# zyang1580/PDA

Hardware: AMD Instinct MI355X
Metric: users/sec full-catalogue top-K@50 (eval) (higher is better)
Workload: dtype f32; 1 GPU; C3: synthetic 1000000 users x 200000 items, d=128, PDA condition ((elu+1)*pop^0.22) head, masked top-K@50; ranks_seen=1

## Files before the change

include/pda_hip_experimental.h:

```cpp
#ifndef PDA_HIP_EXPERIMENTAL_H
#define PDA_HIP_EXPERIMENTAL_H

#include "pda_hip.h"

#ifdef __cplusplus
extern "C" {
#endif

int pda_score_topk_huge_splits(int n_users_blk, int n_items_local, int d);

int pda_topk_kth_value(const uint64_t* keys, int n_splits, int n_users_blk, int K, int pos, float* out, void* stream);
int pda_topk_remap_items(uint64_t* keys, size_t n_keys, const int32_t* gid, int n_gid, void* stream);
int pda_topk_seed_bounds(const uint64_t* keys, int n_splits, int n_users_blk, int K, int m, float* bounds, void* stream);
int pda_topk_seed_counts(const uint64_t* keys, int n_splits, int n_users_blk, int K, const float* bounds, int n_thr, int32_t* counts,
                         void* stream);
int pda_topk_seed_pick(const float* bounds, const int32_t* counts, int n_thr, int n_users_blk, int K, float* seed, void* stream);
int pda_topk_seed_refine(const uint64_t* keys, int n_splits, int n_users_blk, int K, float* lo, float* hi, float* mid, int32_t* counts,
                         int mode, void* stream);
int pda_score_topk4_phase_f32(const float* U, const float* I_shard, const void* prep, const float* pop_shard, const int32_t* users,
                              int n_users_blk, int item_offset, int n_items_local, int d, const int64_t* hist_indptr,
                              const int32_t* hist_indices, int hist_row_mode, int K, int head, int early_stop, int n_splits,
                              int phase, int warm_tiles, const float* seed, uint64_t* out_keys, void* workspace, void* stream);
int pda_score_topk4_phase_bf16(const uint16_t* U, const uint16_t* I_shard, const void* prep, const float* pop_shard,
                               const int32_t* users, int n_users_blk, int item_offset, int n_items_local, int d,
                               const int64_t* hist_indptr, const int32_t* hist_indices, int hist_row_mode, int K, int head,
                               int early_stop, int n_splits, int phase, int warm_tiles, const float* seed, uint64_t* out_keys,
                               void* workspace, void* stream);
int pda_score_topk4_phase_image_offsets(int n_users_blk, int n_items_local, int d, int n_splits, size_t* offs);
int pda_score_topk4_phase_user_image(const void* U, int bf16, const int32_t* users, int n_users_blk, int d, void* ufrag, float* unorm,
                                     void* stream);
int pda_score_topk4_phase_mask_table(const void* prep, int n_items_local, int d, int item_offset, const int64_t* hist_indptr,
                                     const int32_t* hist_indices, int n_rows, uint32_t* table, void* stream);
int pda_score_topk4_phase_masked_f32(const float* U, const float* I_shard, const void* prep, const float* pop_shard, const int32_t* users,
                                     int n_users_blk, int item_offset, int n_items_local, int d, const int64_t* hist_indptr,
                                     const int32_t* hist_indices, int hist_row_mode, int K, int head, int early_stop, int n_splits,
                                     const uint32_t* mask_table, int mask_table_rows, uint64_t* out_keys, void* workspace, void* stream);
int pda_score_topk4_phase_masked_bf16(const uint16_t* U, const uint16_t* I_shard, const void* prep, const float* pop_shard, const int32_t* users,
                                      int n_users_blk, int item_offset, int n_items_local, int d, const int64_t* hist_indptr,
                                      const int32_t* hist_indices, int hist_row_mode, int K, int head, int early_stop, int n_splits,
                                      const uint32_t* mask_table, int mask_table_rows, uint64_t* out_keys, void* workspace, void* stream);
int pda_score_topk4_phase_mask_rows(const void* prep, const int32_t* users, int n_users_blk, int item_offset, int n_items_local, int d,
                                    const int64_t* hist_indptr, const int32_t* hist_indices, int hist_row_mode, int warm_tiles, uint32_t* out,
                                    void* stream);
int pda_score_topk4_phase_mask_offsets(int n_users_blk, int n_items_local, int d, int n_splits, size_t* offs);
#define PDA_SWEEP_WARM_ONE_KERNEL 2048

size_t pda_triplet_plan_bytes(int B);
size_t pda_triplet_plan_large_workspace_bytes(int B);
int pda_triplet_plan_large(const int32_t* users, const int32_t* pos, const int32_t* neg, int B, void* plan, void* workspace, void* stream);
size_t pda_bpr_step_plan_scratch_bytes(int B, int d);
int pda_triplet_plan(const int32_t* users, const int32_t* pos, const int32_t* neg, int B, int n_batches, void* plans, void* stream);
int pda_bpr_step_plan_f32(float* U, float* I, const int32_t* users, const int32_t* pos, const int32_t* neg, const float* pos_pop,
                          const float* neg_pop, int B, int d, float regs, float reg_div, float lr, const void* plan, float* scratch,
                          int exact, float* loss_acc, void* stream);
int pda_bpr_step_plan_bf16(uint16_t* U_bf16, uint16_t* I_bf16, float* U_master, float* I_master, const int32_t* users,
                           const int32_t* pos, const int32_t* neg, const float* pos_pop, const float* neg_pop, int B, int d,
                           float regs, float reg_div, float lr, const void* plan, float* scratch, float* loss_acc, void* stream);

int pda_sort_triplets_by_pos(int32_t* users, int32_t* pos, int32_t* neg, float* pos_pop, float* neg_pop, int B,
                             void* stream);

int pda_group_triplets_by_pos(int32_t* users, int32_t* pos, int32_t* neg, float* pos_pop, float* neg_pop, int B,
                              void* stream);

int pda_adam_mark_rows(const int32_t* users, const int32_t* pos, const int32_t* neg, int B, uint32_t* touched_u, uint32_t* touched_i, void* stream);
int pda_adam_dense_sweep3_f32(float* var_a, float* m_a, float* v_a, float* g_a, size_t rows_a, uint32_t* touched_a, float* var_b, float* m_b, float* v_b,
                              float* g_b, size_t rows_b, uint32_t* touched_b, int d, float lr_t, float beta1, float beta2, float eps, void* stream);

int pda_adam_rows_f32(float* var, float* m, float* v, float* g, const int32_t* rows, int n_rows, int d, float lr_t,
                      float beta1, float beta2, float eps, void* stream);

int pda_adam_lazy_f32(int phase, float* U, float* mU, float* vU, float* gU, int32_t* lastU, float* I, float* mI, float* vI,
                      float* gI, int32_t* lastI, const int32_t* users, const int32_t* pos, const int32_t* neg, int B, int d, int t,
                      const float* lr_tab, float beta1, float beta2, float eps, void* stream);
int pda_adam_lazy_sync_f32(float* var, float* m, float* v, int32_t* last, size_t n_rows, int d, int t, const float* lr_tab,
                           float beta1, float beta2, float eps, void* stream);
int pda_adam_lazy_dev_f32(int phase, float* U, float* mU, float* vU, float* gU, int32_t* lastU, float* I, float* mI, float* vI,
// ... 42 lines not shown
```

pda_amd/_lib.py:

```python
from __future__ import annotations

import ctypes as C
import os

_HERE = os.path.dirname(os.path.abspath(__file__))
LIB_PATH = os.environ.get("PDA_HIP_LIB") or os.path.join(_HERE, "csrc", "libpda_hip.so")

ABI_VERSION = 2
HEAD_RAW, HEAD_POP = 0, 1
HIST_BY_BLOCK_ROW, HIST_BY_USER_ID = 0, 1
UPD_NONE, UPD_SGD_FUSED, UPD_DENSE_GRAD = 0, 1, 2
UPD_ANY_ORDER = 0x100
UPD_USERS_DISTINCT = 0x200
ADAM_REPLAY_FAST = 0x10
MAX_K = 64
TOPK_CAP = 60

_vp, _i, _f, _u64, _sz = C.c_void_p, C.c_int, C.c_float, C.c_uint64, C.c_size_t

class ScorePlan(C.Structure):
    _fields_ = [("path", _i), ("sweep_mode", _i), ("n_splits", _i), ("early_stop", _i), ("order", _i), ("prep_with_pop", _i),
                ("workspace_bytes", _sz), ("keys_rows", _sz)]


# ... 24 lines not shown
    "pda_item_prep_bf16": (_i, [_vp, _i, _i, _vp, _vp]),
    "pda_score_topk_bf16": (_i, [_vp, _vp, _vp, _vp, _vp, _i, _i, _i, _i, _vp, _vp, _i, _i, _i, _i, _vp, _vp, _vp]),
    "pda_item_prep_ordered_bf16_bytes": (_sz, [_i, _i]),
    "pda_item_prep_ordered_bf16": (_i, [_vp, _vp, _vp, _i, _i, _vp, _vp]),
    "pda_score_topk_ordered_bf16": (_i, [_vp, _vp, _vp, _vp, _vp, _i, _i, _i, _i, _vp, _vp, _vp, _i, _i, _i, _i, _i, _vp, _vp, _vp]),
    "pda_item_prep4_bytes": (_sz, [_i, _i]),
    "pda_item_prep4_f32": (_i, [_vp, _vp, _vp, _i, _i, _vp, _vp]),
    "pda_item_prep4_bf16": (_i, [_vp, _vp, _vp, _i, _i, _vp, _vp]),
    "pda_item_prep7_f32": (_i, [_vp, _vp, _i, _i, _vp, _vp]),
    "pda_item_prep7_bf16": (_i, [_vp, _vp, _i, _i, _vp, _vp]),
    "pda_item_prep4_check": (_i, [_vp, _i, _i, _vp]),
    "pda_score_topk4_auto_splits": (_i, [_i, _i, _i]),
    "pda_score_topk4_f32": (_i, [_vp, _vp, _vp, _vp, _vp, _i, _i, _i, _i, _vp, _vp, _i, _i, _i, _i, _i, _vp, _vp, _vp]),
    "pda_score_topk4_bf16": (_i, [_vp, _vp, _vp, _vp, _vp, _i, _i, _i, _i, _vp, _vp, _i, _i, _i, _i, _i, _vp, _vp, _vp]),
    "pda_peak_mfma_flops_per_launch": (C.c_double, [_i]),
    "pda_peak_mfma_bf16": (_i, [_vp, _i, _vp]),
    "pda_peak_mfma_bf16_const": (_i, [_vp, _i, _vp]),
    "pda_peak_mfma_lds_flops_per_launch": (C.c_double, [_i]),
    "pda_peak_mfma_lds_bf16": (_i, [_vp, _sz, _vp, _i, _vp]),
    "pda_peak_copy": (_i, [_vp, _vp, _sz, _vp]),
    "pda_topk_kth_value": (_i, [_vp, _i, _i, _i, _i, _vp, _vp]),
    "pda_topk_remap_items": (_i, [_vp, _sz, _vp, _i, _vp]),
    "pda_topk_seed_refine": (_i, [_vp, _i, _i, _i, _vp, _vp, _vp, _vp, _i, _vp]),
    "pda_topk_seed_bounds": (_i, [_vp, _i, _i, _i, _i, _vp, _vp]),
    "pda_topk_seed_counts": (_i, [_vp, _i, _i, _i, _vp, _i, _vp, _vp]),
    "pda_topk_seed_pick": (_i, [_vp, _vp, _i, _i, _i, _vp, _vp]),
    "pda_score_topk4_phase_f32": (_i, [_vp, _vp, _vp, _vp, _vp, _i, _i, _i, _i, _vp, _vp, _i, _i, _i, _i, _i, _i, _i, _vp, _vp, _vp, _vp]),
    "pda_score_topk4_phase_bf16": (_i, [_vp, _vp, _vp, _vp, _vp, _i, _i, _i, _i, _vp, _vp, _i, _i, _i, _i, _i, _i, _i, _vp, _vp, _vp, _vp]),
    "pda_score_topk4_phase_image_offsets": (_i, [_i, _i, _i, _i, _vp]),
    "pda_score_topk4_phase_user_image": (_i, [_vp, _i, _vp, _i, _i, _vp, _vp, _vp]),
    "pda_score_topk4_phase_mask_table": (_i, [_vp, _i, _i, _i, _vp, _vp, _i, _vp, _vp]),
    "pda_score_topk4_phase_mask_rows": (_i, [_vp, _vp, _i, _i, _i, _i, _vp, _vp, _i, _i, _vp, _vp]),
    "pda_score_topk4_phase_mask_offsets": (_i, [_i, _i, _i, _i, _vp]),
    "pda_score_topk4_phase_masked_f32": (_i, [_vp, _vp, _vp, _vp, _vp, _i, _i, _i, _i, _vp, _vp, _i, _i, _i, _i, _i, _vp, _i, _vp, _vp, _vp]),
    "pda_score_topk4_phase_masked_bf16": (_i, [_vp, _vp, _vp, _vp, _vp, _i, _i, _i, _i, _vp, _vp, _i, _i, _i, _i, _i, _vp, _i, _vp, _vp, _vp]),
    "pda_score_topk_plan": (_i, [_i, _i, _i, _i, _i, _i, _i, _i, _vp]),
    "pda_score_topk_huge_splits": (_i, [_i, _i, _i]),
    "pda_score_topk7_workspace_bytes": (_sz, [_i, _i, _i]),
    "pda_score_topk7_f32": (_i, [_vp, _vp, _vp, _vp, _i, _i, _i, _i, _vp, _vp, _i, _i, _i, _vp, _vp, _vp]),
    "pda_score_topk7_bf16": (_i, [_vp, _vp, _vp, _vp, _i, _i, _i, _i, _vp, _vp, _i, _i, _i, _vp, _vp, _vp]),
    "pda_topk_merge": (_i, [_vp, _i, _i, _i, _vp, _vp, _vp, _vp, _vp, _vp, _i, _vp]),
    "pda_bpr_step_f32": (_i, [_vp, _vp, _vp, _vp, _vp, _vp, _vp, _i, _i, _f, _f, _f, _i, _vp, _vp, _vp, _vp, _vp, _vp, _vp]),
    "pda_triplet_plan_bytes": (_sz, [_i]),
    "pda_bpr_step_plan_scratch_bytes": (_sz, [_i, _i]),
    "pda_triplet_plan": (_i, [_vp, _vp, _vp, _i, _i, _vp, _vp]),
    "pda_triplet_plan_large_workspace_bytes": (_sz, [_i]),
    "pda_triplet_plan_large": (_i, [_vp, _vp, _vp, _i, _vp, _vp, _vp]),
    "pda_bpr_step_plan_f32": (_i, [_vp, _vp, _vp, _vp, _vp, _vp, _vp, _i, _i, _f, _f, _f, _vp, _vp, _i, _vp, _vp]),
    "pda_bpr_step_plan_bf16": (_i, [_vp, _vp, _vp, _vp, _vp, _vp, _vp, _vp, _vp, _i, _i, _f, _f, _f, _vp, _vp, _vp, _vp]),
    "pda_sgd_apply_f32": (_i, [_vp, _vp, _vp, _vp, _vp, _vp, _vp, _vp, _i, _i, _f, _vp]),
    "pda_bpr_step_shard_f32": (_i, [_vp, _vp, _i, _vp, _vp, _vp, _vp, _vp, _i, _i, _f, _f, _f, _f, _vp, _i, _vp, _vp, _vp]),
    "pda_apply_user_grads_f32": (_i, [_vp, _vp, _vp, _i, _i, _i, _f, _vp]),
    "pda_bpr_step_bf16": (_i, [_vp, _vp, _vp, _vp, _vp, _vp, _vp, _vp, _vp, _i, _i, _f, _f, _f, _i, _vp, _vp, _vp, _vp, _vp, _vp, _vp]),
    "pda_refresh_rows_bf16": (_i, [_vp, _vp, _vp, _i, _i, _vp]),
    "pda_group_triplets_by_pos": (_i, [_vp, _vp, _vp, _vp, _vp, _i, _vp]),
    "pda_sort_triplets_by_pos": (_i, [_vp, _vp, _vp, _vp, _vp, _i, _vp]),
    "pda_adam_dense_sweep_f32": (_i, [_vp, _vp, _vp, _vp, _sz, _f, _f, _f, _f, _vp]),
    "pda_adam_dense_sweep2_f32": (_i, [_vp, _vp, _vp, _vp, _sz, _vp, _vp, _vp, _vp, _sz, _f, _f, _f, _f, _vp]),
    "pda_adam_mark_rows": (_i, [_vp, _vp, _vp, _i, _vp, _vp, _vp]),
    "pda_adam_dense_sweep3_f32": (_i, [_vp, _vp, _vp, _vp, _sz, _vp, _vp, _vp, _vp, _vp, _sz, _vp, _i, _f, _f, _f, _f, _vp]),
    "pda_score_dense_f32": (_i, [_vp, _vp, _vp, _vp, _i, _vp, _i, _i, _i, _vp, _vp]),
    "pda_adam_dense_sweep4_f32": (_i, [_vp, _vp, _vp, _vp, _sz, _vp, _vp, _vp, _vp, _vp, _sz, _vp, _i, _i, _f, _f, _f, _f, _i, _vp]),
    "pda_adam_step_f32": (_i, [_vp, _vp, _vp, _vp, _vp, _sz, _vp, _vp, _vp, _vp, _vp, _sz, _vp, _vp, _vp, _vp, _vp, _i, _i, _f, _f, _i, _f, _f, _f, _f,
                               _i, _i, _vp, _vp]),
    "pda_adam_rows_f32": (_i, [_vp, _vp, _vp, _vp, _vp, _i, _i, _f, _f, _f, _f, _vp]),
    "pda_adam_lazy_f32": (_i, [_i] + [_vp] * 13 + [_i, _i, _i, _vp, _f, _f, _f, _vp]),
# ... 121 lines not shown
```

pda_amd/csrc/pda_score_topk_v4.hip:

```cpp
#include "pda_v4_shared.h"
#include <cstdlib>
#include <type_traits>

using namespace pda_topk;

namespace {

constexpr int kCap4 = 57;
constexpr int kRing4 = 128;
constexpr int kWarmTiles = 4;
constexpr int kMainWaves = 8;
#ifndef PDA_W4_ABL
#define PDA_W4_ABL 0
#endif
#ifdef PDA_V4_PROF
__device__ unsigned long long pda_prof4[24];
#define PROF_T0(v) const long long v = __builtin_readcyclecounter()
#define PROF_T1(v, slot) prof[slot] += (unsigned long long)(__builtin_readcyclecounter() - v)
#define PROF_INC(slot, x) prof[slot] += (unsigned long long)(x)
#define PROF_FLUSH(first, last) do { if (lane == 0) for (int pq = (first); pq <= (last); ++pq) atomicAdd(&pda_prof4[pq], prof[pq]); } while (0)
#else
#define PROF_T0(v) do {} while (0)
#define PROF_T1(v, slot) do {} while (0)
#define PROF_INC(slot, x) do {} while (0)
// ... 680 lines not shown
        } else if (rb < g.n_users_blk && lane < K) {
            const uint64_t k = lane < c ? buf[lane] : 0ull;
            g.out_keys[((size_t)split * g.n_users_blk + rb) * K + lane] = k;
        }
    }
    if (g.kth_ws != nullptr) {
        pda_wave_sync();
        const int rb0 = utile * kUserTile + wave * 32, nv = max(0, min(32, g.n_users_blk - rb0));
        if (lane < nv) {
            const uint64_t kl = my_lists[(size_t)lane * CAP + (K - 1)];
            g.kth_ws[(size_t)split * g.n_users_blk + rb0 + lane] = cntl[wave * 32 + lane] >= K ? pda_unordf((uint32_t)(kl >> 32)) : -INFINITY;
        }
        uint64_t* ob = g.out_keys + ((size_t)split * g.n_users_blk + rb0) * K;
        const int q64 = 64 / K, r64 = 64 % K;
        int rr = lane / K, p = lane % K;
        for (int i = lane; i < nv * K; i += 64) {
            ob[i] = p < cntl[wave * 32 + rr] ? my_lists[(size_t)rr * CAP + p] : 0ull;
            rr += q64;
            p += r64;
            if (p >= K) { p -= K; ++rr; }
        }
    }
    if (g.pred_ws != nullptr && lane < 32) {
        const int rb = utile * kUserTile + wave * 32 + lane;
        if (rb < g.n_users_blk) {
            g.pred_ws[2 * (size_t)rb] = predt[wave * 32 + lane];
            g.pred_ws[2 * (size_t)rb + 1] = nul[wave * 32 + lane];
        }
    }
}

constexpr int kWS5Waves = 8, kWS5Threads = 64 * kWS5Waves;
constexpr int kWarmPos = 64 * kWarmTiles;
constexpr size_t warm_score5_lds(int d) { return (size_t)kWarmPos * d * 4 + kWarmPos * 8 + (size_t)kWS5Waves * 32 * 2 * kWarmTiles * 4; }

template <int D, bool BF>
__global__ void __launch_bounds__(kWS5Threads) warm_score5_kernel(Args4 g) {
    extern __shared__ __attribute__((aligned(16))) unsigned char smem[];
    constexpr int RB = row_bytes(D);
    constexpr int NC = D / 8;
    constexpr int CPR4 = D / 4;
    float* Bt = reinterpret_cast<float*>(smem);
    float* popw = Bt + kWarmPos * D;
    int* idw = reinterpret_cast<int*>(popw + kWarmPos);
    unsigned* hmask = reinterpret_cast<unsigned*>(idw + kWarmPos);

    const int tid = threadIdx.x, lane = tid & 63, wave = tid >> 6;
    const int j = lane & 31, h = lane >> 5;
    const int nwarm = g.warm_tiles;
    const int npos = 64 * nwarm;
    for (int p = tid; p < npos; p += kWS5Threads) {
        const float* tl = reinterpret_cast<const float*>(g.rows + (size_t)p * RB + 2 * D + 32);
        popw[p] = tl[0];
        idw[p] = reinterpret_cast<const int*>(tl)[1];
    }
    __syncthreads();
    for (int id = tid; id < npos * CPR4; id += kWS5Threads) {
        const int jj = id / CPR4, ch = id % CPR4;
        *reinterpret_cast<f32x4*>(Bt + jj * D + 4 * (ch ^ swz<D>(jj & 31))) = pda_load4<BF>(g.I, (size_t)idw[jj] * D + 4 * ch);
    }
    if (blockIdx.x == 0) {
        for (int p = tid; p < kWarmPos; p += kWS5Threads) g.wscore[p] = p < npos ? (uint32_t)idw[p] : 0u;
        if (tid == 0) g.stats[8] = 5u;
    }
    __syncthreads();

    uint32_t* scores = g.wscore + kWarmPos;
    const int utiles_w = (g.n_users_blk + kUserTile - 1) / kUserTile;
    const int nunits = utiles_w * (kUserTile / 32);
    const int G = (int)gridDim.x, stride = G * kWS5Waves;
    unsigned* hm_l = hmask + wave * 32 * 2 * kWarmTiles;
    static_assert(2 * kWarmTiles == 8, "two 16-byte loads per row");

    auto row_uid = [&](int unit) -> int {
        const int rb = unit * 32 + j;
        return (unit < nunits && rb < g.n_users_blk) ? g.users[rb] : 0;
    };
    auto load_rows = [&](int unit_x, int uid, f32x4 (&a)[NC], u32x4& hm, bool& hm_on) __attribute__((always_inline)) {
        if (unit_x >= nunits) return;
        const int rb = unit_x * 32 + j;
#pragma unroll
        for (int c = 0; c < NC; ++c) a[c] = pda_load4<BF>(g.U, (size_t)uid * D + 4 * h + 8 * c);
        hm_on = false;
        if (g.hmask_tab != nullptr) {
            hm_on = rb < g.n_users_blk && (unsigned)uid < (unsigned)g.hmask_tab_rows;
            hm = *reinterpret_cast<const u32x4*>(g.hmask_tab + (size_t)(hm_on ? uid : 0) * (2 * kWarmTiles) + 4 * h);
        } else if (g.hmask_ws != nullptr) {
            hm_on = true;
            hm = *reinterpret_cast<const u32x4*>(g.hmask_ws + (size_t)rb * (2 * kWarmTiles) + 4 * h);
        }
    };
    unsigned long long n_tiles_done = 0ull;
    auto run_unit = [&](const int unit_in, f32x4 (&areg)[NC], const u32x4& hm_in, const bool hm_on) __attribute__((always_inline)) {
        const int unit = __builtin_amdgcn_readfirstlane(unit_in);
        const int row_blk = unit * 32 + j;
        if (unit * 32 + 32 > g.n_users_blk) {
            const f32x4 z = {0.f, 0.f, 0.f, 0.f};
#pragma unroll
            for (int c = 0; c < NC; ++c) areg[c] = row_blk < g.n_users_blk ? areg[c] : z;
        }
        const u32x4 hz = {0u, 0u, 0u, 0u};
        const u32x4 hmv = hm_on ? hm_in : hz;
        *reinterpret_cast<u32x4*>(hm_l + j * (2 * kWarmTiles) + 4 * h) = hmv;
        {
            constexpr int NK5 = D / 32;
            unsigned char* fb = g.ufrag_out + ((size_t)(row_blk >> 4) * (NK5 * 64) + (size_t)(row_blk & 15)) * 16 + 8 * h;
            float ssc[NC];
#pragma unroll
            for (int c = 0; c < NC; ++c) {
                const f32x4 v = areg[c];
                uint2 w;
                w.x = bf16_rne(v[0]) | (bf16_rne(v[1]) << 16);
                w.y = bf16_rne(v[2]) | (bf16_rne(v[3]) << 16);
                *reinterpret_cast<uint2*>(fb + ((c >> 2) * 64 + 16 * (c & 3)) * 16) = w;
                float ss = 0.f;
#pragma unroll
                for (int k = 0; k < 4; ++k) {
                    const float sq = v[k] * v[k];
                    ss += sq + __shfl_xor(sq, 32, 64);
                }
                ssc[c] = ss;
                __builtin_amdgcn_sched_barrier(0);
            }
#pragma unroll
            for (int o = NC / 2; o > 0; o >>= 1)
#pragma unroll
                for (int c = 0; c < o; ++c) ssc[c] += ssc[c + o];
            if (h == 0) g.unorm_out[row_blk] = sqrtf(ssc[0]) * 1.0009765625f * 1.0001f;
        }
        if ((unit & (kUserTile / 32 - 1)) == 0) n_tiles_done += (unsigned long long)(2 * nwarm);
        pda_wave_sync();
        const int j_lane = j, h_lane = h;
#pragma unroll 1
        for (int ht = 0; ht < 2 * nwarm; ++ht) {
            int j = j_lane, h = h_lane;
#if defined(__HIP_DEVICE_COMPILE__)
            asm volatile("" : "+v"(j), "+v"(h));
#endif
            const int bswz = swz<D>(j);
            const float* brow = Bt + (ht * 32 + j) * D;
            f32x16 acc0 = zero16v(), acc1 = zero16v();
            f32x4 b0 = *reinterpret_cast<const f32x4*>(brow + 4 * (h ^ bswz));
            f32x4 b1 = *reinterpret_cast<const f32x4*>(brow + 4 * ((2 + h) ^ bswz));
#pragma unroll
            for (int c = 0; c < NC; c += 2) {
                f32x4 n0 = b0, n1 = b1;
                if (c + 2 < NC) {
                    n0 = *reinterpret_cast<const f32x4*>(brow + 4 * ((2 * c + 4 + h) ^ bswz));
                    n1 = *reinterpret_cast<const f32x4*>(brow + 4 * ((2 * c + 6 + h) ^ bswz));
                }
#pragma unroll
                for (int q = 0; q < 4; ++q) {
                    acc0 = __builtin_amdgcn_mfma_f32_32x32x2f32(areg[c][q], b0[q], acc0, 0, 0, 0);
                    acc1 = __builtin_amdgcn_mfma_f32_32x32x2f32(areg[c + 1][q], b1[q], acc1, 0, 0, 0);
                }
                __builtin_amdgcn_sched_barrier(0);
                b0 = n0;
                b1 = n1;
            }
            const f32x16 accx = acc0 + acc1;
            const bool okw = (ht * 32 + j) < g.n_items_local;
            const float pv = popw[ht * 32 + j];
            const unsigned hb_mine = hm_l[j * (2 * kWarmTiles) + ht];
            const bool any_hb = __any(hb_mine != 0u);
            const uint32_t soff = (uint32_t)(unit * 32 + 4 * h) * (uint32_t)npos + (uint32_t)(ht * 32 + j);
#pragma unroll
            for (int r = 0; r < 16; ++r) {
                const int row = (r & 3) + 8 * (r >> 2) + 4 * h;
                float sc = accx[r];
                sc = (sc > 0.0f ? sc + 1.0f : __expf(sc)) * pv;
                bool p = okw && (sc >= -INFINITY);
                if (any_hb) {
                    const uint32_t hbr = (uint32_t)__shfl((int)hb_mine, row, 64);
                    if ((hbr >> j) & 1u) p = false;
                }
                scores[soff + (uint32_t)((r & 3) + 8 * (r >> 2)) * (uint32_t)npos] = p ? pda_ordf(sc + 0.0f) : 0u;
            }
        }
        pda_wave_sync();
    };
    int unit = (int)blockIdx.x + G * wave;
    f32x4 ra[NC], rb_[NC];
    u32x4 ha = {0u, 0u, 0u, 0u}, hb = {0u, 0u, 0u, 0u};
    bool oa = false, ob = false;
    load_rows(unit, row_uid(unit), ra, ha, oa);
    int uid_n = row_uid(unit + stride);
    while (unit < nunits) {
        load_rows(unit + stride, uid_n, rb_, hb, ob);
        uid_n = row_uid(unit + 2 * stride);
        run_unit(unit, ra, ha, oa);
        unit += stride;
        if (unit >= nunits) break;
        load_rows(unit + stride, uid_n, ra, ha, oa);
        uid_n = row_uid(unit + 2 * stride);
        run_unit(unit, rb_, hb, ob);
        unit += stride;
    }
    if (lane == 0 && n_tiles_done != 0ull) atomicAdd(reinterpret_cast<unsigned long long*>(g.stats + 2), n_tiles_done);
    if ((int)blockIdx.x == (nunits - 1) % G) {
        const size_t r0 = (size_t)utiles_w * kUserTile, r1 = ((size_t)g.n_users_blk + kUT5 - 1) / kUT5 * kUT5;
        const u32x4 z = {0u, 0u, 0u, 0u};
        for (size_t q = r0 * (2 * D) + (size_t)tid * 16; q < r1 * (2 * D); q += (size_t)kWS5Threads * 16) *reinterpret_cast<u32x4*>(g.ufrag_out + q) = z;
        for (size_t r = r0 + tid; r < r1; r += kWS5Threads) g.unorm_out[r] = 0.f;
    }
}

constexpr int kSelRows = 16;
__global__ void __launch_bounds__(256) __attribute__((amdgpu_waves_per_eu(8))) warm_select5_kernel(Args4 g) {
    constexpr int CAP = kCap4;
    __shared__ uint64_t lists[4][2][64];
    const int tid = threadIdx.x, lane = tid & 63, wave = tid >> 6;
    const int K = g.K, n = g.n_users_blk;
    const int npos = 64 * g.warm_tiles;
    const uint32_t* scores = g.wscore + kWarmPos;
    const int rb0 = ((int)blockIdx.x * 4 + wave) * kSelRows;
    if (rb0 >= n) return;
    const u32x4 idv = *reinterpret_cast<const u32x4*>(g.wscore + 4 * lane);
    uint32_t klo[4];
#pragma unroll
    for (int q = 0; q < 4; ++q) klo[q] = 0xFFFFFFFFu - (uint32_t)(g.item_offset + (int)idv[q]);
    const bool lane_on = 4 * lane < npos;
    float kth_mine = -INFINITY;

    auto count32 = [&](const u32x4& v, uint32_t t) __attribute__((always_inline)) -> int {
        return __popcll(__ballot(v[0] >= t)) + __popcll(__ballot(v[1] >= t)) + __popcll(__ballot(v[2] >= t)) + __popcll(__ballot(v[3] >= t));
    };
    auto key_of = [&](const u32x4& v, int q) __attribute__((always_inline)) -> uint64_t { return ((uint64_t)v[q] << 32) | (uint64_t)klo[q]; };
    auto count64 = [&](const u32x4& v, uint64_t t) __attribute__((always_inline)) -> int {
        int c = 0;
#pragma unroll
        for (int q = 0; q < 4; ++q) c += __popcll(__ballot(key_of(v, q) >= t));
        return c;
    };

#pragma unroll 1
    for (int it = 0; it < kSelRows; it += 2) {
        if (rb0 + it >= n) break;
        u32x4 v[2];
        uint32_t t[2], hi[2];
        int ct[2];
        bool need[2];
#pragma unroll
        for (int s = 0; s < 2; ++s) {
            const int rb = rb0 + it + s;
            const u32x4 z = {0u, 0u, 0u, 0u};
            v[s] = (lane_on && rb < n) ? *reinterpret_cast<const u32x4*>(scores + (size_t)rb * npos + 4 * lane) : z;
        }
#pragma unroll
        for (int s = 0; s < 2; ++s) {
            ct[s] = count32(v[s], 1u);
            t[s] = 1u;
            hi[s] = 0u;
            need[s] = ct[s] > CAP;
        }
        if (need[0] || need[1]) {
#pragma unroll
            for (int s = 0; s < 2; ++s) {
                uint32_t mx = max(max(v[s][0], v[s][1]), max(v[s][2], v[s][3])), mn = 0xFFFFFFFFu;
#pragma unroll
                for (int q = 0; q < 4; ++q) mn = min(mn, v[s][q] != 0u ? v[s][q] : 0xFFFFFFFFu);
#pragma unroll
                for (int o = 32; o >= 1; o >>= 1) {
                    mx = max(mx, (uint32_t)__shfl_xor((int)mx, o, 64));
                    mn = min(mn, (uint32_t)__shfl_xor((int)mn, o, 64));
                }
                hi[s] = (uint32_t)__builtin_amdgcn_readfirstlane((int)mx) + 1u;
                if (need[s]) t[s] = (uint32_t)__builtin_amdgcn_readfirstlane((int)mn);
            }
            for (int step = 0; step < 40; ++step) {
                const bool open0 = need[0] && ct[0] > CAP && hi[0] - t[0] > 1u;
                const bool open1 = need[1] && ct[1] > CAP && hi[1] - t[1] > 1u;
                if (!(open0 || open1)) break;
                const uint32_t mid0 = open0 ? t[0] + ((hi[0] - t[0]) >> 1) : t[0];
                const uint32_t mid1 = open1 ? t[1] + ((hi[1] - t[1]) >> 1) : t[1];
                const int c0 = count32(v[0], mid0), c1 = count32(v[1], mid1);
                if (open0) {
                    if (c0 >= K) { t[0] = mid0; ct[0] = c0; } else { hi[0] = mid0; }
                }
                if (open1) {
                    if (c1 >= K) { t[1] = mid1; ct[1] = c1; } else { hi[1] = mid1; }
// ... 1081 lines not shown
    }
    if (c.sweep != Call4::kSweep4) return PDA_ERR_ARG;
    return launch_sweep4<D, HEAD, BF, 0>(g, c, stream);
}

int user_tile4(int d) { return d == 64 ? Geo4<64>::UT : d == 128 ? Geo4<128>::UT : Geo4<256>::UT; }
struct Ws4 {
    size_t lists, bloom, hmask, regroup, handover, ufrag, unorm, seed, kth, wscore, total;
};
static Ws4 ws4_layout(int n_users_blk, int d, int n_splits) {
    auto al = [](size_t x) { return (x + 255) & ~(size_t)255; };
    Ws4 w{};
    w.lists = al(pda_score_topk_workspace_bytes(n_users_blk));
    size_t b = w.lists;
    const size_t ut = 1024;
    b += ((size_t)n_users_blk + ut - 1) / ut * (size_t)n_splits * ut * kCap4 * 8 + 256;
    w.bloom = al(b);
    w.hmask = al(w.bloom + (size_t)n_users_blk * 128);
    w.regroup = al(w.hmask + ((size_t)n_users_blk + kUserTile - 1) / kUserTile * (size_t)n_splits * kUserTile * 2 * kWarmTiles * 4);
    w.handover = al(w.regroup + (1024 + 4 * (size_t)n_users_blk) * 4);
    w.total = w.handover + (size_t)n_splits * (size_t)n_users_blk * kCap4 * 8;
    w.ufrag = al(w.total);
    w.unorm = w.ufrag;
    {
        const size_t n_pad = ((size_t)n_users_blk + kUT5 - 1) / kUT5 * kUT5;
        w.unorm = w.ufrag + al(n_pad * 2 * (size_t)d);
        w.total = w.unorm + al(n_pad * 4);
    }
    w.seed = w.total;
    w.total = w.seed + al((size_t)n_users_blk * 4);
    w.kth = w.total;
    w.total = w.kth + al((size_t)n_splits * (size_t)n_users_blk * 4);
    w.wscore = w.total;
    w.total = w.wscore + al((size_t)kWarmPos * 4 + ((size_t)n_users_blk + kUserTile - 1) / kUserTile * kUserTile * kWarmPos * 4);
    return w;
}
extern "C" size_t pda_score_topk4_workspace_bytes(int n_users_blk, int n_items_local, int d, int n_splits) {
    if (n_users_blk <= 0 || n_items_local <= 0 || (d != 64 && d != 128 && d != 256)) return 0;
    if (n_splits <= 0) n_splits = pda_score_topk4_auto_splits(n_users_blk, n_items_local, d);
    return ws4_layout(n_users_blk, d, n_splits).total;
}

int run_score4(const void* U, const void* I_shard, bool bf16, const void* prep, const float* pop_shard, const int32_t* users,
               int n_users_blk, int item_offset, int n_items_local, int d, const int64_t* hist_indptr, const int32_t* hist_indices,
               int hist_row_mode, int K, int head, int early_stop, int n_splits, uint64_t* out_keys, void* workspace, hipStream_t s,
               int phase = 3, const float* seed = nullptr, int warm_tiles = 0, const int* n_users_dev = nullptr,
               const uint32_t* mask_table = nullptr, int mask_table_rows = 0) {
    if (!U || !I_shard || !prep || !users || !out_keys || !workspace) return PDA_ERR_ARG;
    if (n_users_blk <= 0 || n_items_local <= 0 || item_offset < 0) return PDA_ERR_ARG;
    if (K < 1 || K > PDA_MAX_K) return PDA_ERR_ARG;
    if (early_stop < 0 || (early_stop & ~0xFFF) != 0) return PDA_ERR_ARG;
    const bool warm_per_split = (early_stop & PDA_SWEEP_WARM_PER_SPLIT) != 0;
    const bool warm_one_kernel = (early_stop & PDA_SWEEP_WARM_ONE_KERNEL) != 0;
    int geometry = (early_stop & PDA_SWEEP_HUGE) ? 4 : (early_stop & PDA_SWEEP_MANY_CANDIDATES) ? 3 : 0;
    if (warm_tiles == 0) warm_tiles = (early_stop >> 4) & 7;
    early_stop &= 1;
    if (head != PDA_HEAD_RAW && head != PDA_HEAD_POP) return PDA_ERR_ARG;
    if (head == PDA_HEAD_POP && !pop_shard) return PDA_ERR_ARG;
    if (hist_indptr && !hist_indices) return PDA_ERR_ARG;
    if (d != 64 && d != 128 && d != 256) return PDA_ERR_UNSUPPORTED;
    if (K > kCap4 - 3) return PDA_ERR_UNSUPPORTED;
    if ((uint64_t)n_items_local > (1ull << 26)) return PDA_ERR_UNSUPPORTED;
    if (warm_tiles < 0 || warm_tiles > kWarmTiles) return PDA_ERR_ARG;
    if (warm_tiles == 0) warm_tiles = kWarmTiles;
    const bool from_empty = phase == 4;
    if (from_empty) {
        if (seed == nullptr) return PDA_ERR_ARG;
// ... 374 lines not shown
    g.n_tiles = L.n_tiles;
    g.warm_tiles = warm_tiles;
    return g;
}
extern "C" int pda_score_topk4_phase_mask_table(const void* prep, int n_items_local, int d, int item_offset, const int64_t* hist_indptr,
                                                const int32_t* hist_indices, int n_rows, uint32_t* table, void* stream) {
    if (!prep || !hist_indptr || !hist_indices || !table || n_rows <= 0 || n_items_local <= 0 || item_offset < 0) return PDA_ERR_ARG;
    if (d != 64 && d != 128 && d != 256) return PDA_ERR_UNSUPPORTED;
    const Args4 g = mask_args4(prep, nullptr, n_rows, item_offset, n_items_local, d, hist_indptr, hist_indices, PDA_HIST_BY_BLOCK_ROW, kWarmTiles);
    hipLaunchKernelGGL(warm_mask_table4_kernel, dim3((unsigned)((n_rows + kUserTile - 1) / kUserTile)), dim3(kThreads), 0, reinterpret_cast<hipStream_t>(stream), g, table);
    PDA_CHECK_LAUNCH();
    return PDA_OK;
}
extern "C" int pda_score_topk4_phase_mask_rows(const void* prep, const int32_t* users, int n_users_blk, int item_offset, int n_items_local, int d,
                                               const int64_t* hist_indptr, const int32_t* hist_indices, int hist_row_mode, int warm_tiles, uint32_t* out,
                                               void* stream) {
    if (!prep || !users || !hist_indptr || !hist_indices || !out || n_users_blk <= 0 || n_items_local <= 0 || item_offset < 0) return PDA_ERR_ARG;
    if (warm_tiles < 1 || warm_tiles > kWarmTiles) return PDA_ERR_ARG;
    if (d != 64 && d != 128 && d != 256) return PDA_ERR_UNSUPPORTED;
    const Args4 g = mask_args4(prep, users, n_users_blk, item_offset, n_items_local, d, hist_indptr, hist_indices, hist_row_mode, warm_tiles);
    hipLaunchKernelGGL(warm_mask4_kernel, dim3((unsigned)((n_users_blk + kUserTile - 1) / kUserTile)), dim3(kThreads), 0, reinterpret_cast<hipStream_t>(stream), g, out);
    PDA_CHECK_LAUNCH();
    return PDA_OK;
}
extern "C" int pda_score_topk4_phase_mask_offsets(int n_users_blk, int n_items_local, int d, int n_splits, size_t* offs) {
    if (n_users_blk <= 0 || n_items_local <= 0 || (d != 64 && d != 128 && d != 256) || !offs) return PDA_ERR_ARG;
    if (n_splits <= 0) n_splits = pda_score_topk4_auto_splits(n_users_blk, n_items_local, d);
    const Ws4 W = ws4_layout(n_users_blk, d, n_splits);
    offs[0] = W.hmask;
    offs[1] = W.regroup - W.hmask;
    return PDA_OK;
}

extern "C" int pda_score_topk4_phase_image_offsets(int n_users_blk, int n_items_local, int d, int n_splits, size_t* offs) {
    if (n_users_blk <= 0 || n_items_local <= 0 || (d != 64 && d != 128 && d != 256) || !offs) return PDA_ERR_ARG;
    if (n_splits <= 0) n_splits = pda_score_topk4_auto_splits(n_users_blk, n_items_local, d);
    const Ws4 W = ws4_layout(n_users_blk, d, n_splits);
    const size_t ut = d == 256 ? 512 : kUT5;
    offs[0] = W.ufrag;
    offs[1] = W.unorm;
    offs[2] = W.kth;
    offs[3] = ((size_t)n_users_blk + ut - 1) / ut * ut;
    return PDA_OK;
}
extern "C" int pda_score_topk4_phase_user_image(const void* U, int bf16, const int32_t* users, int n_users_blk, int d, void* ufrag, float* unorm,
                                                void* stream) {
    if (!U || !users || !ufrag || !unorm || n_users_blk <= 0) return PDA_ERR_ARG;
    if (d != 64 && d != 128 && d != 256) return PDA_ERR_UNSUPPORTED;
    hipStream_t s = reinterpret_cast<hipStream_t>(stream);
    const size_t ut = d == 256 ? 512 : kUT5, n_pad = ((size_t)n_users_blk + ut - 1) / ut * ut;
#define PDA_UIMG_(DD, BFV, UPWV)                                                                                                                \
    hipLaunchKernelGGL((uprep5_kernel<DD, BFV, true, UPWV>), dim3((unsigned)((n_pad * (DD / 8) + 255) / 256)), dim3(256), 0, s, U, users, n_users_blk, \
                       (int)n_pad, reinterpret_cast<unsigned char*>(ufrag), unorm)
    if (d == 64) { if (bf16) PDA_UIMG_(64, true, 256); else PDA_UIMG_(64, false, 256); }
    else if (d == 128) { if (bf16) PDA_UIMG_(128, true, 256); else PDA_UIMG_(128, false, 256); }
    else { if (bf16) PDA_UIMG_(256, true, 128); else PDA_UIMG_(256, false, 128); }
#undef PDA_UIMG_
    PDA_CHECK_LAUNCH();
    return PDA_OK;
}
```

pda_amd/csrc/pda_v5_sweep.h:

```cpp
#pragma once
#ifdef PDA_V6_LOOP_HEADER
#include PDA_V6_LOOP_HEADER
#else
#include "pda_v6_loop_asm.h"
#endif
#include "pda_v6_free_asm.h"

#ifdef PDA_V5_EXITPROF
constexpr int kXpMaxWg = 4096;
__device__ unsigned long long pda_v5_exitprof[kXpMaxWg * 4 * 8];
#define XP(...) __VA_ARGS__
#else
#define XP(...)
#endif
constexpr int kRing5 = 192;



template <int D, bool BF, bool S16, int UPW>
__global__ void __launch_bounds__(256, 1) sweep5_kernel(Args4 g) {
    static_assert(slot_bytes5(D) == Loop6<D, 8>::kSlotBytes, "one LDS image for all loops");
    static_assert(S16, "the loop on v_mfma_f32_32x32x16_bf16 (round 4's first form: 9.16 against 8.07 ms, profiles/README.md) left with round 5; the parameter keeps the kernel's name");
    static_assert((D <= 128 && UPW == 256) || (D == 256 && UPW == 128), "users per wave: 256, or (d = 256) 128 -- 8 blocks x 8 k-steps = 256 AGPRs, one 512-user workgroup per CU");
    constexpr int NK = D / 32, UBW = 16, NU = UPW / UBW;
    constexpr int SS = slot_bytes5(D), UT = 4 * UPW, CAPL = kCap4, RB4 = row_bytes(D);
    constexpr int LPC = D / 32, CPP = 64 / LPC;
    constexpr float kEps5 = BF ? 4.0234375e-3f : 8.046875e-3f;
    extern __shared__ __attribute__((aligned(16))) unsigned char smem[];
    unsigned char* tiles = smem;
    int* cntl = reinterpret_cast<int*>(smem + kNSlot5 * SS);
    float* taul = reinterpret_cast<float*>(cntl + UT);
    uint64_t* crings = reinterpret_cast<uint64_t*>(taul + UT);
    unsigned* sync = reinterpret_cast<unsigned*>(crings + 4 * kRing5);
    unsigned* s_uns = sync + 8;
    unsigned* touched = sync + 40;
    const int tid = threadIdx.x, lane = tid & 63;
    const int wave = __builtin_amdgcn_readfirstlane(tid >> 6);
    const int split = blockIdx.x % g.n_splits, utile = blockIdx.x / g.n_splits;
    XP(unsigned long long xp[8] = {0, 0, 0, 0, 0, 0, 0, 0}; const unsigned long long xp_k0 = wall_clock64(); unsigned long long xp_out = 0, xp_re = 0;)
    uint64_t* lists = g.handover != nullptr ? g.handover + ((size_t)split * g.n_users_blk + (size_t)utile * UT) * kCap4
                                            : g.lists_ws + (size_t)blockIdx.x * UT * CAPL;
    const int K = g.K;
    const int nt = split_tiles(g.n_tiles, split, g.n_splits);
    const int wt = warm_tiles_of(g, split);
    const bool starts_empty = g.lists_empty || (g.warm_shared && split > 0);
    const bool warm_final = g.warm_final && !starts_empty;
    const int n_it = max(0, nt - wt);
    const unsigned hend = 2u * (unsigned)n_it;
// ... 307 lines not shown
                if (b + 1 < NB) load_cur(bn);
                if (__any(mm != 0ull)) {
#pragma unroll 1
                    for (int q = 0; q < 2 * BU; ++q) {
                        uint32_t m = (uint32_t)(mm >> (NR * q)) & ((1u << NR) - 1u);
                        const int u = b * BU + (q >> 1);
                        const unsigned pos0 = (q & 1) ? pos01 : pos00;
                        while (__any(m != 0u)) {
                            if (ring_n + 64u > (unsigned)kRing5) {
                                rescore_ring();
                                if constexpr (AF_ONCE) {
                                    load_af(0);
                                    load_af(1);
                                }
                                load_cur(bn);
                            }
                            const bool act = m != 0u;
                            const int r = __builtin_ctz(m | 0x10000u);
                            m &= ~(1u << r);
                            const uint64_t pm = __ballot(act);
                            const unsigned slot = ring_n + (unsigned)__builtin_amdgcn_mbcnt_hi((uint32_t)(pm >> 32), __builtin_amdgcn_mbcnt_lo((uint32_t)pm, 0));
                            if (act) my_ring[slot] = ((uint64_t)(unsigned)(UBW * u + j) << 32) | (uint64_t)(pos0 + item_of(r));
                            ring_n += (unsigned)__popcll(pm);
                        }
                    }
                }
            }
        };

        auto decided = [&](float tw, float nw, unsigned h_now) __attribute__((always_inline)) -> unsigned {
#ifdef PDA_V5_NO_FREE
            return hend;
#else
            if (g.tailA == nullptr || !(tw > -1.0e30f)) return hend;
            int lo = (int)(h_now >> 1), hi = n_it;
            while (lo < hi) {
                const int mid = (lo + hi) >> 1;
                const size_t T = (size_t)t0 + (size_t)mid * (size_t)g.n_splits;
                if (__builtin_fmaf(nw, g.tailB[T], g.tailA[T]) * 1.000002f < tw) hi = mid; else lo = mid + 1;
            }
            return 2u * (unsigned)lo;
#endif
        };
        float* xch = reinterpret_cast<float*>(sync + 72);
        unsigned h = 0, issued = 0, n_entries = 0, n_free = 0;
        unsigned hlim = hend;
        bool hend_ok = true;
        if ((ring_lds & (D == 256 ? 511u : 255u)) != 0u) { if (lane == 0) g.stats[0] = 6u; hend_ok = false; }
        for (unsigned guard = 0; hend_ok && guard < 2u * hend + 8u; ++guard) {
            float thr[NU];
#pragma unroll
            for (int u = 0; u < NU; ++u) thr[u] = thr_of(u);
            unsigned reason = 0;
            float tmin = thr[0];
#pragma unroll
            for (int u = 1; u < NU; ++u) tmin = fminf(tmin, thr[u]);
#pragma unroll
            for (int o = 32; o >= 1; o >>= 1) tmin = fminf(tmin, __shfl_xor(tmin, o, 64));
            tmin = __int_as_float(__builtin_amdgcn_readfirstlane(__float_as_int(tmin)));
            if (lane == 0) { xch[wave] = tmin; xch[4 + wave] = numax; }
            __syncthreads();
            const float tw = __int_as_float(__builtin_amdgcn_readfirstlane(__float_as_int(fminf(fminf(xch[0], xch[1]), fminf(xch[2], xch[3])))));
            const float nw = __int_as_float(__builtin_amdgcn_readfirstlane(__float_as_int(fmaxf(fmaxf(xch[4], xch[5]), fmaxf(xch[6], xch[7])))));
            const unsigned hf = decided(tw, nw, h);
            if (h >= min(hlim, hf)) {
                if (h > hlim) h = hlim;
                if (issued > hlim) issued = hlim;
                if (h < hend) {
                    ++n_entries;
                    n_free = hend - h;
                    XP(if (xp_out != 0) { const unsigned long long t_ = wall_clock64(); xp[3] += t_ - xp_out; xp[2] += t_ - xp_re; xp_out = 0; } else xp[6] = wall_clock64() - xp_k0;)
                    Loop6Free<D, NU>::run(h, issued, hend, ring_lds, 1024u * (unsigned)wave, t0, (unsigned)g.n_splits, (unsigned)img, (unsigned)(img >> 32), my_ufrag, lane16);
                }
                break;
// ... 112 lines not shown
```

Measured before the change: 34.42 million users/s.

## Move warm-tile head and history masking into select; widen decided search across wave

The warm scoring kernel now writes raw dot products and no longer applies the (elu+1)*pop head or the history mask. It also drops its per-wave mask staging in LDS and the wave syncs around it. The select kernel instead reads popularity and mask bits per lane and applies the head while loading scores. Separately, the binary search for the decided tile in the sweep loop becomes a 64-way wave-parallel search using ballot, and a permlane32 swap replaces a cross-half shuffle. A small test entry point for the search is added. Risks: expf work moves into select and masks are loaded once per row there, and the wave search issues more memory loads per step.

Measured after the change: 34.64 million users/s (median of 6 runs). No clear change (+0.6%).

```diff
diff --git a/include/pda_hip_experimental.h b/include/pda_hip_experimental.h
--- a/include/pda_hip_experimental.h
+++ b/include/pda_hip_experimental.h
@@ -43,6 +43,8 @@
                                     const int64_t* hist_indptr, const int32_t* hist_indices, int hist_row_mode, int warm_tiles, uint32_t* out,
                                     void* stream);
 int pda_score_topk4_phase_mask_offsets(int n_users_blk, int n_items_local, int d, int n_splits, size_t* offs);
+int pda_score_topk4_phase_decided_search(const float* tailA, const float* tailB, int t0, int n_splits, int n_it, const int32_t* h_now,
+                                         const float* nw, const float* tw, int n_q, int32_t* out, void* stream);
 #define PDA_SWEEP_WARM_ONE_KERNEL 2048
 
 size_t pda_triplet_plan_bytes(int B);
diff --git a/pda_amd/_lib.py b/pda_amd/_lib.py
--- a/pda_amd/_lib.py
+++ b/pda_amd/_lib.py
@@ -80,6 +80,7 @@
     "pda_score_topk4_phase_mask_table": (_i, [_vp, _i, _i, _i, _vp, _vp, _i, _vp, _vp]),
     "pda_score_topk4_phase_mask_rows": (_i, [_vp, _vp, _i, _i, _i, _i, _vp, _vp, _i, _i, _vp, _vp]),
     "pda_score_topk4_phase_mask_offsets": (_i, [_i, _i, _i, _i, _vp]),
+    "pda_score_topk4_phase_decided_search": (_i, [_vp, _vp, _i, _i, _i, _vp, _vp, _vp, _i, _vp, _vp]),
     "pda_score_topk4_phase_masked_f32": (_i, [_vp, _vp, _vp, _vp, _vp, _i, _i, _i, _i, _vp, _vp, _i, _i, _i, _i, _i, _vp, _i, _vp, _vp, _vp]),
     "pda_score_topk4_phase_masked_bf16": (_i, [_vp, _vp, _vp, _vp, _vp, _i, _i, _i, _i, _vp, _vp, _i, _i, _i, _i, _i, _vp, _i, _vp, _vp, _vp]),
     "pda_score_topk_plan": (_i, [_i, _i, _i, _i, _i, _i, _i, _i, _vp]),
diff --git a/pda_amd/csrc/pda_score_topk_v4.hip b/pda_amd/csrc/pda_score_topk_v4.hip
--- a/pda_amd/csrc/pda_score_topk_v4.hip
+++ b/pda_amd/csrc/pda_score_topk_v4.hip
@@ -736,7 +736,16 @@
 
 constexpr int kWS5Waves = 8, kWS5Threads = 64 * kWS5Waves;
 constexpr int kWarmPos = 64 * kWarmTiles;
-constexpr size_t warm_score5_lds(int d) { return (size_t)kWarmPos * d * 4 + kWarmPos * 8 + (size_t)kWS5Waves * 32 * 2 * kWarmTiles * 4; }
+constexpr size_t warm_score5_lds(int d) { return (size_t)kWarmPos * d * 4 + kWarmPos * 4; }
+
+__device__ __forceinline__ float other_half(float x, int h) {
+#if defined(__HIP_DEVICE_COMPILE__)
+    const auto sw = __builtin_amdgcn_permlane32_swap(__float_as_uint(x), __float_as_uint(x), false, false);
+    return __uint_as_float(h ? sw[0] : sw[1]);
+#else
+    return x;
+#endif
+}
 
 template <int D, bool BF>
 __global__ void __launch_bounds__(kWS5Threads) warm_score5_kernel(Args4 g) {
@@ -745,9 +754,7 @@
     constexpr int NC = D / 8;
     constexpr int CPR4 = D / 4;
     float* Bt = reinterpret_cast<float*>(smem);
-    float* popw = Bt + kWarmPos * D;
-    int* idw = reinterpret_cast<int*>(popw + kWarmPos);
-    unsigned* hmask = reinterpret_cast<unsigned*>(idw + kWarmPos);
+    int* idw = reinterpret_cast<int*>(Bt + kWarmPos * D);
 
     const int tid = threadIdx.x, lane = tid & 63, wave = tid >> 6;
     const int j = lane & 31, h = lane >> 5;
@@ -755,8 +762,8 @@
     const int npos = 64 * nwarm;
     for (int p = tid; p < npos; p += kWS5Threads) {
         const float* tl = reinterpret_cast<const float*>(g.rows + (size_t)p * RB + 2 * D + 32);
-        popw[p] = tl[0];
         idw[p] = reinterpret_cast<const int*>(tl)[1];
+        if (blockIdx.x == 0) g.wscore[kWarmPos + p] = __float_as_uint(tl[0]);
     }
     __syncthreads();
     for (int id = tid; id < npos * CPR4; id += kWS5Threads) {
@@ -764,38 +771,30 @@
         *reinterpret_cast<f32x4*>(Bt + jj * D + 4 * (ch ^ swz<D>(jj & 31))) = pda_load4<BF>(g.I, (size_t)idw[jj] * D + 4 * ch);
     }
     if (blockIdx.x == 0) {
-        for (int p = tid; p < kWarmPos; p += kWS5Threads) g.wscore[p] = p < npos ? (uint32_t)idw[p] : 0u;
+        for (int p = tid; p < kWarmPos; p += kWS5Threads) {
+            g.wscore[p] = p < npos ? (uint32_t)idw[p] : 0u;
+            if (p >= npos) g.wscore[kWarmPos + p] = 0u;
+        }
         if (tid == 0) g.stats[8] = 5u;
     }
     __syncthreads();
 
-    uint32_t* scores = g.wscore + kWarmPos;
+    float* scores = reinterpret_cast<float*>(g.wscore + 2 * kWarmPos);
     const int utiles_w = (g.n_users_blk + kUserTile - 1) / kUserTile;
     const int nunits = utiles_w * (kUserTile / 32);
     const int G = (int)gridDim.x, stride = G * kWS5Waves;
-    unsigned* hm_l = hmask + wave * 32 * 2 * kWarmTiles;
-    static_assert(2 * kWarmTiles == 8, "two 16-byte loads per row");
 
     auto row_uid = [&](int unit) -> int {
         const int rb = unit * 32 + j;
         return (unit < nunits && rb < g.n_users_blk) ? g.users[rb] : 0;
     };
-    auto load_rows = [&](int unit_x, int uid, f32x4 (&a)[NC], u32x4& hm, bool& hm_on) __attribute__((always_inline)) {
+    auto load_rows = [&](int unit_x, int uid, f32x4 (&a)[NC]) __attribute__((always_inline)) {
         if (unit_x >= nunits) return;
-        const int rb = unit_x * 32 + j;
 #pragma unroll
         for (int c = 0; c < NC; ++c) a[c] = pda_load4<BF>(g.U, (size_t)uid * D + 4 * h + 8 * c);
-        hm_on = false;
-        if (g.hmask_tab != nullptr) {
-            hm_on = rb < g.n_users_blk && (unsigned)uid < (unsigned)g.hmask_tab_rows;
-            hm = *reinterpret_cast<const u32x4*>(g.hmask_tab + (size_t)(hm_on ? uid : 0) * (2 * kWarmTiles) + 4 * h);
-        } else if (g.hmask_ws != nullptr) {
-            hm_on = true;
-            hm = *reinterpret_cast<const u32x4*>(g.hmask_ws + (size_t)rb * (2 * kWarmTiles) + 4 * h);
-        }
     };
     unsigned long long n_tiles_done = 0ull;
-    auto run_unit = [&](const int unit_in, f32x4 (&areg)[NC], const u32x4& hm_in, const bool hm_on) __attribute__((always_inline)) {
+    auto run_unit = [&](const int unit_in, f32x4 (&areg)[NC]) __attribute__((always_inline)) {
         const int unit = __builtin_amdgcn_readfirstlane(unit_in);
         const int row_blk = unit * 32 + j;
         if (unit * 32 + 32 > g.n_users_blk) {
@@ -803,9 +802,6 @@
 #pragma unroll
             for (int c = 0; c < NC; ++c) areg[c] = row_blk < g.n_users_blk ? areg[c] : z;
         }
-        const u32x4 hz = {0u, 0u, 0u, 0u};
-        const u32x4 hmv = hm_on ? hm_in : hz;
-        *reinterpret_cast<u32x4*>(hm_l + j * (2 * kWarmTiles) + 4 * h) = hmv;
         {
             constexpr int NK5 = D / 32;
             unsigned char* fb = g.ufrag_out + ((size_t)(row_blk >> 4) * (NK5 * 64) + (size_t)(row_blk & 15)) * 16 + 8 * h;
@@ -821,7 +817,7 @@
 #pragma unroll
                 for (int k = 0; k < 4; ++k) {
                     const float sq = v[k] * v[k];
-                    ss += sq + __shfl_xor(sq, 32, 64);
+                    ss += sq + other_half(sq, h);
                 }
                 ssc[c] = ss;
                 __builtin_amdgcn_sched_barrier(0);
@@ -833,7 +829,6 @@
             if (h == 0) g.unorm_out[row_blk] = sqrtf(ssc[0]) * 1.0009765625f * 1.0001f;
         }
         if ((unit & (kUserTile / 32 - 1)) == 0) n_tiles_done += (unsigned long long)(2 * nwarm);
-        pda_wave_sync();
         const int j_lane = j, h_lane = h;
 #pragma unroll 1
         for (int ht = 0; ht < 2 * nwarm; ++ht) {
@@ -863,41 +858,25 @@
                 b1 = n1;
             }
             const f32x16 accx = acc0 + acc1;
-            const bool okw = (ht * 32 + j) < g.n_items_local;
-            const float pv = popw[ht * 32 + j];
-            const unsigned hb_mine = hm_l[j * (2 * kWarmTiles) + ht];
-            const bool any_hb = __any(hb_mine != 0u);
-            const uint32_t soff = (uint32_t)(unit * 32 + 4 * h) * (uint32_t)npos + (uint32_t)(ht * 32 + j);
-#pragma unroll
-            for (int r = 0; r < 16; ++r) {
-                const int row = (r & 3) + 8 * (r >> 2) + 4 * h;
-                float sc = accx[r];
-                sc = (sc > 0.0f ? sc + 1.0f : __expf(sc)) * pv;
-                bool p = okw && (sc >= -INFINITY);
-                if (any_hb) {
-                    const uint32_t hbr = (uint32_t)__shfl((int)hb_mine, row, 64);
-                    if ((hbr >> j) & 1u) p = false;
-                }
-                scores[soff + (uint32_t)((r & 3) + 8 * (r >> 2)) * (uint32_t)npos] = p ? pda_ordf(sc + 0.0f) : 0u;
-            }
-        }
-        pda_wave_sync();
+            const uint32_t soff = (uint32_t)(unit * 32 + 4 * h) * (uint32_t)kWarmPos + (uint32_t)(ht * 32 + j);
+            float* const srow = scores + soff;
+#pragma unroll
+            for (int r = 0; r < 16; ++r) srow[((r & 3) + 8 * (r >> 2)) * kWarmPos] = accx[r];
+        }
     };
     int unit = (int)blockIdx.x + G * wave;
     f32x4 ra[NC], rb_[NC];
-    u32x4 ha = {0u, 0u, 0u, 0u}, hb = {0u, 0u, 0u, 0u};
-    bool oa = false, ob = false;
-    load_rows(unit, row_uid(unit), ra, ha, oa);
+    load_rows(unit, row_uid(unit), ra);
     int uid_n = row_uid(unit + stride);
     while (unit < nunits) {
-        load_rows(unit + stride, uid_n, rb_, hb, ob);
+        load_rows(unit + stride, uid_n, rb_);
         uid_n = row_uid(unit + 2 * stride);
-        run_unit(unit, ra, ha, oa);
+        run_unit(unit, ra);
         unit += stride;
         if (unit >= nunits) break;
-        load_rows(unit + stride, uid_n, ra, ha, oa);
+        load_rows(unit + stride, uid_n, ra);
         uid_n = row_uid(unit + 2 * stride);
-        run_unit(unit, rb_, hb, ob);
+        run_unit(unit, rb_);
         unit += stride;
     }
     if (lane == 0 && n_tiles_done != 0ull) atomicAdd(reinterpret_cast<unsigned long long*>(g.stats + 2), n_tiles_done);
@@ -916,14 +895,42 @@
     const int tid = threadIdx.x, lane = tid & 63, wave = tid >> 6;
     const int K = g.K, n = g.n_users_blk;
     const int npos = 64 * g.warm_tiles;
-    const uint32_t* scores = g.wscore + kWarmPos;
+    const uint32_t* scores = g.wscore + 2 * kWarmPos;
     const int rb0 = ((int)blockIdx.x * 4 + wave) * kSelRows;
     if (rb0 >= n) return;
+    const f32x4 popv = *reinterpret_cast<const f32x4*>(g.wscore + kWarmPos + 4 * lane);
+    uint32_t gone = 0u;
+#pragma unroll
+    for (int q = 0; q < 4; ++q) gone |= (4 * lane + q < npos && 4 * lane + q < g.n_items_local) ? 0u : (1u << q);
+    const int mword = lane >> 3, mshift = 4 * (lane & 7);
+    int uid_l = 0;
+    if (g.hmask_tab != nullptr && lane < kSelRows && rb0 + lane < n) uid_l = g.users[rb0 + lane];
+    auto drop_of = [&](int rb, int row_w) __attribute__((always_inline)) -> uint32_t {
+        if (rb >= n) return 15u;
+        uint32_t mw = 0u;
+        if (g.hmask_tab != nullptr) {
+            const int uid = __builtin_amdgcn_readlane(uid_l, row_w);
+            if ((unsigned)uid < (unsigned)g.hmask_tab_rows) mw = g.hmask_tab[(size_t)uid * (2 * kWarmTiles) + mword];
+        } else if (g.hmask_ws != nullptr) {
+            mw = g.hmask_ws[(size_t)rb * (2 * kWarmTiles) + mword];
+        }
+        return ((mw >> mshift) & 15u) | gone;
+    };
+    auto head_of = [&](const u32x4& raw, uint32_t drop) __attribute__((always_inline)) -> u32x4 {
+        u32x4 o;
+#pragma unroll
+        for (int q = 0; q < 4; ++q) {
+            float sc = __uint_as_float(raw[q]);
+            sc = (sc > 0.0f ? sc + 1.0f : __expf(sc)) * popv[q];
+            const bool p = (sc >= -INFINITY) && ((drop >> q) & 1u) == 0u;
+            o[q] = p ? pda_ordf(sc + 0.0f) : 0u;
+        }
+        return o;
+    };
     const u32x4 idv = *reinterpret_cast<const u32x4*>(g.wscore + 4 * lane);
     uint32_t klo[4];
 #pragma unroll
     for (int q = 0; q < 4; ++q) klo[q] = 0xFFFFFFFFu - (uint32_t)(g.item_offset + (int)idv[q]);
-    const bool lane_on = 4 * lane < npos;
     float kth_mine = -INFINITY;
 
     auto count32 = [&](const u32x4& v, uint32_t t) __attribute__((always_inline)) -> int {
@@ -944,12 +951,16 @@
         uint32_t t[2], hi[2];
         int ct[2];
         bool need[2];
+        uint32_t drop[2];
 #pragma unroll
         for (int s = 0; s < 2; ++s) {
             const int rb = rb0 + it + s;
             const u32x4 z = {0u, 0u, 0u, 0u};
-            v[s] = (lane_on && rb < n) ? *reinterpret_cast<const u32x4*>(scores + (size_t)rb * npos + 4 * lane) : z;
-        }
+            v[s] = (gone != 15u && rb < n) ? *reinterpret_cast<const u32x4*>(scores + (size_t)rb * kWarmPos + 4 * lane) : z;
+            drop[s] = drop_of(rb, it + s);
+        }
+#pragma unroll
+        for (int s = 0; s < 2; ++s) v[s] = head_of(v[s], drop[s]);
 #pragma unroll
         for (int s = 0; s < 2; ++s) {
             ct[s] = count32(v[s], 1u);
@@ -2097,7 +2108,7 @@
     w.kth = w.total;
     w.total = w.kth + al((size_t)n_splits * (size_t)n_users_blk * 4);
     w.wscore = w.total;
-    w.total = w.wscore + al((size_t)kWarmPos * 4 + ((size_t)n_users_blk + kUserTile - 1) / kUserTile * kUserTile * kWarmPos * 4);
+    w.total = w.wscore + al((size_t)2 * kWarmPos * 4 + ((size_t)n_users_blk + kUserTile - 1) / kUserTile * kUserTile * kWarmPos * 4);
     return w;
 }
 extern "C" size_t pda_score_topk4_workspace_bytes(int n_users_blk, int n_items_local, int d, int n_splits) {
@@ -2538,6 +2549,29 @@
     return PDA_OK;
 }
 
+__global__ void __launch_bounds__(64) decided_search_kernel(const float* tailA, const float* tailB, int t0, int n_splits, int n_it, const int32_t* h_now,
+                                                            const float* nw, const float* tw, int n_q, int32_t* out) {
+    const unsigned lane = threadIdx.x;
+    for (int q = 0; q < n_q; ++q) {
+        const unsigned h = (unsigned)__builtin_amdgcn_readfirstlane(h_now[q]);
+        const float n = __int_as_float(__builtin_amdgcn_readfirstlane(__float_as_int(nw[q])));
+        const float t = __int_as_float(__builtin_amdgcn_readfirstlane(__float_as_int(tw[q])));
+        const unsigned a = decided_halftile<true>(tailA, tailB, (unsigned)t0, (unsigned)n_splits, h, n_it, n, t, lane);
+        const unsigned b = decided_halftile<false>(tailA, tailB, (unsigned)t0, (unsigned)n_splits, h, n_it, n, t, lane);
+        if (lane == 0) {
+            out[2 * q] = (int32_t)a;
+            out[2 * q + 1] = (int32_t)b;
+        }
+    }
+}
+extern "C" int pda_score_topk4_phase_decided_search(const float* tailA, const float* tailB, int t0, int n_splits, int n_it, const int32_t* h_now,
+                                                    const float* nw, const float* tw, int n_q, int32_t* out, void* stream) {
+    if (!tailB || !h_now || !nw || !tw || !out || t0 < 0 || n_splits < 1 || n_it < 0 || n_q <= 0) return PDA_ERR_ARG;
+    hipLaunchKernelGGL(decided_search_kernel, dim3(1), dim3(64), 0, reinterpret_cast<hipStream_t>(stream), tailA, tailB, t0, n_splits, n_it, h_now, nw, tw, n_q, out);
+    PDA_CHECK_LAUNCH();
+    return PDA_OK;
+}
+
 extern "C" int pda_score_topk4_phase_image_offsets(int n_users_blk, int n_items_local, int d, int n_splits, size_t* offs) {
     if (n_users_blk <= 0 || n_items_local <= 0 || (d != 64 && d != 128 && d != 256) || !offs) return PDA_ERR_ARG;
     if (n_splits <= 0) n_splits = pda_score_topk4_auto_splits(n_users_blk, n_items_local, d);
diff --git a/pda_amd/csrc/pda_v5_sweep.h b/pda_amd/csrc/pda_v5_sweep.h
--- a/pda_amd/csrc/pda_v5_sweep.h
+++ b/pda_amd/csrc/pda_v5_sweep.h
@@ -14,6 +14,36 @@
 #define XP(...)
 #endif
 constexpr int kRing5 = 192;
+
+__device__ __forceinline__ int decided_tile_scalar(const float* tailA, const float* tailB, unsigned t0, unsigned n_splits, int lo, int n_it, float nw, float tw) {
+    int hi = n_it;
+    while (lo < hi) {
+        const int mid = (lo + hi) >> 1;
+        const size_t T = (size_t)t0 + (size_t)mid * (size_t)n_splits;
+        if (__builtin_fmaf(nw, tailB[T], tailA[T]) * 1.000002f < tw) hi = mid; else lo = mid + 1;
+    }
+    return lo;
+}
+__device__ __forceinline__ int decided_tile_wave(const float* tailA, const float* tailB, unsigned t0, unsigned n_splits, int lo, int n_it, float nw, float tw, unsigned lane) {
+    int hi = n_it;
+    while (lo < hi) {
+        const int step = (hi - lo + 63) >> 6;
+        const int m = min(lo + ((int)lane + 1) * step - 1, hi - 1);
+        const size_t T = (size_t)t0 + (size_t)m * (size_t)n_splits;
+        const unsigned long long yes = __ballot(__builtin_fmaf(nw, tailB[T], tailA[T]) * 1.000002f < tw);
+        if (yes == 0ull) return hi;
+        const int f = __builtin_ctzll(yes);
+        hi = min(lo + (f + 1) * step - 1, hi - 1);
+        lo = lo + f * step;
+    }
+    return lo;
+}
+template <bool WAVE>
+__device__ __forceinline__ unsigned decided_halftile(const float* tailA, const float* tailB, unsigned t0, unsigned n_splits, unsigned h_now, int n_it, float nw, float tw, unsigned lane) {
+    if (tailA == nullptr || !(tw > -1.0e30f)) return 2u * (unsigned)n_it;
+    const int lo = (int)(h_now >> 1);
+    return 2u * (unsigned)(WAVE ? decided_tile_wave(tailA, tailB, t0, n_splits, lo, n_it, nw, tw, lane) : decided_tile_scalar(tailA, tailB, t0, n_splits, lo, n_it, nw, tw));
+}
 
 
 
@@ -387,14 +417,7 @@
 #ifdef PDA_V5_NO_FREE
             return hend;
 #else
-            if (g.tailA == nullptr || !(tw > -1.0e30f)) return hend;
-            int lo = (int)(h_now >> 1), hi = n_it;
-            while (lo < hi) {
-                const int mid = (lo + hi) >> 1;
-                const size_t T = (size_t)t0 + (size_t)mid * (size_t)g.n_splits;
-                if (__builtin_fmaf(nw, g.tailB[T], g.tailA[T]) * 1.000002f < tw) hi = mid; else lo = mid + 1;
-            }
-            return 2u * (unsigned)lo;
+            return decided_halftile<true>(g.tailA, g.tailB, t0, (unsigned)g.n_splits, h_now, n_it, nw, tw, (unsigned)lane);
 #endif
         };
         float* xch = reinterpret_cast<float*>(sync + 72);
```
